# strawberrylady99/mythril

Measured on AMD Instinct MI355X. Metric: candidate assignments evaluated/sec (node) + time-to-first-model vs z3, higher is better.
Workload: dtype u32

## Files before the change

mythril_amd/csrc/jit_asm.cpp:

```cpp
#include <algorithm>
#include <array>
#include <cstdio>
#include <cstring>
#include <functional>
#include <map>
#include <set>
#include <sstream>
#include <string>
#include <vector>

#include "jit.hpp"

namespace mg {

namespace {

struct AsmFail {
  std::string why;
};
[[noreturn]] void fail(const std::string& w) { throw AsmFail{w}; }

inline uint32_t Lw(uint32_t w) { return (w + 31) / 32; }
inline uint32_t topmask(uint32_t w) { return (w & 31) ? ((1u << (w & 31)) - 1u) : 0xFFFFFFFFu; }
inline uint32_t gsalt(uint32_t c, uint32_t j) { return c * 0x9E3779B9u + j * 0x85EBCA6Bu + 0x27D4EB2Fu; }
// ... 134 lines not shown
  }
  std::function<bool()> on_pressure;
  std::function<bool()> on_hard;
  int vsoft = 256;
  int vhard = 256;
  uint32_t valloc() {
    for (;;) {
      int r = vfirst;
      while (r < vhard && vref[r]) r++;
      if ((r >= 256 || r >= vsoft) && on_pressure && on_pressure()) continue;
      if (r >= vhard && on_hard && on_hard()) continue;
      if (r >= vhard) fail("out of VGPRs");
      if (lds_pending.count(r)) lds_flush();
      vref[r] = 1;
      vgen[r] = ++gen_ctr;
      vhigh = std::max(vhigh, r + 1);
      return (uint32_t)r;
    }
  }
  uint32_t valloc2() {
    for (;;) {
      int r = (vfirst + 1) & ~1;
      while (r + 1 < vhard && (vref[r] || vref[r + 1])) r += 2;
      if ((r + 1 >= 256 || r + 1 >= vsoft) && on_pressure && on_pressure()) continue;
      if (r + 1 >= vhard && on_hard && on_hard()) continue;
      if (r + 1 >= vhard) fail("out of VGPRs");
      if (lds_pending.count(r) || lds_pending.count(r + 1)) lds_flush();
      for (int q = 0; q < 2; q++) {
        vref[r + q] = 1;
        vgen[r + q] = ++gen_ctr;
      }
      vhigh = std::max(vhigh, r + 2);
      return (uint32_t)r;
    }
  }
  void retain(const Limb& l) {
    check(l);
    if (l.reg() && (int)l.v >= vfirst) vref[l.v]++;
  }
  std::function<void(uint32_t)> on_free;
  void release(const Limb& l) {
    check(l);
    if (l.reg() && (int)l.v >= vfirst) {
      if (--vref[l.v] < 0) fail("internal: VGPR released twice");
      if (vref[l.v] == 0 && on_free) on_free(vgen[l.v]);
    }
  }
  int sfree() const {
    int n = 0;
    for (int r = kS0; r + 1 < kS1; r += 2) n += !sref[r];
    return n;
  }
  std::function<bool()> on_spressure;
  int salloc() {
    for (;;) {
      for (int r = kS0; r + 1 < kS1; r += 2)
        if (!sref[r]) {
          sref[r] = 1;
          shigh = std::max(shigh, r + 2);
          return r;
        }
      if (!on_spressure || !on_spressure()) break;
    }
    fail("out of SGPRs");
  }
  void sretain(const Mask& m) {
    if (m.k == 2) sref[m.s]++;
  }
  void srelease(const Mask& m) {
    if (m.k == 2 && --sref[m.s] < 0) fail("internal: SGPR pair released twice");
  }
};

struct Gen {
  const Lowered& P;
  const std::vector<GenSpec>& specs;
  const std::vector<uint32_t>& G;
  mutable Emitter E;
  std::vector<Val> val;
  std::vector<uint64_t> need;
  std::vector<int32_t> last;
  std::map<uint32_t, uint32_t> cval;
  std::vector<int32_t> def;
  std::vector<uint32_t> copysrc;
  bool gen_kernel = false;
  bool eval_kernel = false;
  std::map<uint32_t, uint32_t> lds_base;
  std::map<uint32_t, std::pair<uint32_t, uint32_t>> lds_shape;
  uint32_t lds_words = 0;
  static constexpr uint32_t kLdsWords = 8192;

  std::vector<Instr> code;
  Gen(const Lowered& p, const std::vector<GenSpec>& s, const std::vector<uint32_t>& g)
      : P(p), specs(s), G(g), val(p.vwidth.size()), need(p.vwidth.size(), 0), last(p.vwidth.size(), -1),
        def(p.vwidth.size(), -1), code(p.vcode) {}

  void reorder() {
    const std::vector<Instr>& v = P.vcode;
    std::vector<int32_t> dix(P.vwidth.size(), -1);
    for (size_t k = 0; k < v.size(); k++)
      if (v[k].dst != MG_NONE && v[k].dst < dix.size() && dix[v[k].dst] < 0) dix[v[k].dst] = (int32_t)k;
    std::map<uint32_t, int32_t> coord_at;
    for (size_t k = 0; k < v.size(); k++)
      if (v[k].op == K_COORD && !coord_at.count(v[k].p0)) coord_at[v[k].p0] = (int32_t)k;
    auto operands = [&](const Instr& in, std::vector<int32_t>& out) {
      out.clear();
      auto add = [&](uint32_t id) {
        if (id != MG_NONE && id < dix.size() && dix[id] >= 0) out.push_back(dix[id]);
      };
      switch (in.op) {
        case K_CONST: break;
// ... 508 lines not shown
      E.ctl("s_waitcnt vmcnt(0)");
      for (auto& pr : pend) {
        E.mem("ds_write_b32 " + VL(pr.second) + ", " + VL(pr.first));
        drop(pr.first);
        drop(pr.second);
      }
      pend.clear();
    };
    for (const auto& kv : lds_base) {
      const uint32_t off = kv.first, base = kv.second, n = lds_shape[off].first, Lc = lds_shape[off].second;
      const uint32_t nL = n * Lc, M = (65536u + Lc - 1) / Lc;
      for (uint32_t it = 0; it * 256 < nL; it++) {
        const Limb vi = fresh(), vt = fresh(), ve = fresh(), vj = fresh();
        E.valu("v_add_u32_e32 " + VL(vi) + ", " + imm(256 * it) + ", v0");
        E.valu("v_min_u32_e32 " + VL(vi) + ", " + imm(nL - 1) + ", " + VL(vi));
        E.valu("v_lshlrev_b32_e32 " + VL(vt) + ", 2, " + VL(vi));
        if (off * 4 < 4096) {
          E.mem("global_load_dword " + VL(vt) + ", " + VL(vt) + ", s[4:5] offset:" + std::to_string(off * 4));
        } else {
          E.valu("v_add_u32_e32 " + VL(vt) + ", " + hexs(off * 4) + ", " + VL(vt));
          E.mem("global_load_dword " + VL(vt) + ", " + VL(vt) + ", s[4:5]");
        }
        E.valu("v_mul_u32_u24_e32 " + VL(ve) + ", " + imm(M) + ", " + VL(vi));
        E.valu("v_lshrrev_b32_e32 " + VL(ve) + ", 16, " + VL(ve));
        E.valu("v_mul_u32_u24_e32 " + VL(vj) + ", " + imm(Lc) + ", " + VL(ve));
        E.valu("v_sub_u32_e32 " + VL(vj) + ", " + VL(vi) + ", " + VL(vj));
        if (lds_pairs()) {
          const Limb vo = fresh();
          E.valu("v_and_b32_e32 " + VL(vo) + ", 1, " + VL(vj));
          E.valu("v_and_b32_e32 " + VL(vj) + ", -2, " + VL(vj));
          E.valu("v_mul_u32_u24_e32 " + VL(vj) + ", " + imm(n) + ", " + VL(vj));
          E.valu("v_lshl_add_u32 " + VL(ve) + ", " + VL(ve) + ", 1, " + VL(vo));
          drop(vo);
        } else {
          E.valu("v_mul_u32_u24_e32 " + VL(vj) + ", " + imm(n) + ", " + VL(vj));
        }
        if (!inl(base)) E.salu("s_mov_b32 s41, " + hexs(base), {41});
        E.valu("v_add3_u32 " + VL(vj) + ", " + VL(vj) + ", " + VL(ve) + ", " + (inl(base) ? imm(base) : "s41"), {41});
        E.valu("v_lshlrev_b32_e32 " + VL(vj) + ", 2, " + VL(vj));
        drop(vi);
        drop(ve);
        pend.push_back({vt, vj});
        if (pend.size() >= stage_batch()) flush();
      }
    }
    flush();
    E.ctl("s_waitcnt lgkmcnt(0)");
    E.ctl("s_barrier");
  }

  Emitter& e() { return E; }

  int cond = 0;
  struct CondScope {
    Gen& g;
    explicit CondScope(Gen& g_) : g(g_) { g.cond++; }
    ~CondScope() { g.cond--; }
  };
  std::map<uint32_t, Limb> litcache;
  uint64_t tick = 0;
  std::map<uint32_t, uint64_t> lit_last;
  std::map<std::pair<uint64_t, uint64_t>, uint64_t> x_last;
  std::map<std::pair<uint32_t, uint32_t>, uint64_t> eq_last;
  void litcache_clear() {
    std::vector<Limb> held;
    for (auto& kv : litcache) held.push_back(kv.second);
    litcache.clear();
    lit_last.clear();
    for (auto& d : held) drop(d);
  }
  Limb vreg(const Limb& l) {
    if (l.reg()) {
      E.retain(l);
      return l;
    }
    const uint32_t x = l.lit() ? l.v : 0u;
    if (x == 0) return Reg(6);
    auto it = pool.find(x);
    if (it != pool.end()) return Reg((uint32_t)it->second);
    const bool cache = !cond && !no_lvn() && lvn_on && caches;
    if (cache) {
      auto c = litcache.find(x);
      if (c != litcache.end()) {
        lit_last[x] = ++tick;
        E.retain(c->second);
        return c->second;
      }
    }
    census[x]++;
    const Limb r = fresh();
    E.valu("v_mov_b32_e32 " + VL(r) + ", " + imm(x));
    if (cache) {
      E.retain(r);
      litcache[x] = r;
      lit_last[x] = ++tick;
    }
    return r;
  }
  bool lvn_on = false;
  bool caches = true;
  int vsoft = 256;
  std::map<uint32_t, int> pool;
  std::map<uint32_t, uint32_t> census;
  std::string src(const Limb& l) const {
    if (l.k == LU) fail("internal: a limb the demand analysis dropped was read");
    E.check(l);
    return l.lit() ? imm(l.v) : VL(l);
  }

// ... 279 lines not shown
    drop(c);
    return d;
  }

  static bool eq_bitop3() {
    static const bool on = [] {
      const char* g = getenv("MYTHGPU_JIT_ASM_EQ_BITOP3");
      return !(g && g[0] == '0');
    }();
    return on;
  }
  struct DLimb {
    uint32_t off = 0, n = 0, Lc = 0, j = 0;
    Limb idx;
  };
  std::map<uint32_t, DLimb> dlimb;
  static bool no_dict_eq() {
    static const bool on = [] {
      const char* g = getenv("MYTHGPU_JIT_ASM_NO_DICT_EQ");
      return g && g[0] == '1';
    }();
    return on;
  }
  void dlimb_free(uint32_t g) {
    auto it = dlimb.find(g);
    if (it == dlimb.end()) return;
    const Limb ix = it->second.idx;
    dlimb.erase(it);
    drop(ix);
  }
  bool dict_limb(const Limb& l, DLimb& out) const {
    if (!l.reg() || !l.g || (int)l.v < E.vfirst || E.vgen[l.v] != l.g) return false;
    auto it = dlimb.find(l.g);
    if (it == dlimb.end()) return false;
    out = it->second;
    return true;
  }
  bool idx_in_set(const Limb& idx, const std::vector<char>& S, uint32_t n, Mask& m) {
    uint32_t cnt = 0, first = 0, miss = 0;
    for (uint32_t e = 0; e < n; e++) {
      if (S[e]) {
        if (!cnt) first = e;
        cnt++;
      } else {
        miss = e;
      }
    }
    if (cnt == 0 || cnt == n) {
      m.k = 1;
      m.ones = cnt == n;
      return true;
    }
    if (cnt != 1 && cnt != n - 1 && n > 32) return false;
    m.k = 2;
    m.s = E.salloc();
    if (cnt == 1 || cnt == n - 1) {
      const uint32_t e = cnt == 1 ? first : miss;
      const std::string op = cnt == 1 ? "v_cmp_eq_u32" : "v_cmp_ne_u32";
      if (inl(e)) {
        E.valu(op + "_e64 " + SP(m.s) + ", " + imm(e) + ", " + VL(idx), {}, {m.s, m.s + 1});
      } else {
        E.valu(op + "_e32 vcc, " + hexs(e) + ", " + VL(idx), {}, {kVCC, kVCC + 1});
        E.salu("s_mov_b64 " + SP(m.s) + ", vcc", {m.s, m.s + 1});
      }
      return true;
    }
    uint32_t bits = 0;
    for (uint32_t e = 0; e < n; e++)
      if (S[e]) bits |= 1u << e;
    const Limb t = fresh();
    E.salu("s_mov_b32 s41, " + hexs(bits), {41});
    E.valu("v_bfe_u32 " + VL(t) + ", s41, " + VL(idx) + ", 1", {41});
    E.valu("v_cmp_ne_u32_e64 " + SP(m.s) + ", 0, " + VL(t), {}, {m.s, m.s + 1});
    drop(t);
    return true;
  }
  bool dict_eq(const std::vector<std::pair<Limb, Limb>>& prs, Mask& m) {
    if (no_dict_eq() || dlimb.empty()) return false;
    bool haveA = false, haveB = false;
    DLimb A, B;
    std::vector<std::pair<uint32_t, uint32_t>> lits;
    std::vector<std::pair<uint32_t, uint32_t>> regs;
    auto same_src = [](const DLimb& x, const DLimb& y) {
      return x.off == y.off && x.n == y.n && x.Lc == y.Lc && x.idx == y.idx && x.idx.g == y.idx.g;
    };
    for (const auto& pr : prs) {
      const Limb a = pr.first, b = pr.second;
      if (a.lit() && b.lit()) {
        if (a.v != b.v) {
          m.k = 1;
          m.ones = false;
          return true;
        }
        continue;
      }
      if (a == b) continue;
      DLimb da, db;
      const bool ia = dict_limb(a, da), ib = dict_limb(b, db);
      if ((ia && b.lit()) || (ib && a.lit())) {
        const DLimb& d = ia ? da : db;
        if (!haveA) {
          A = d;
          haveA = true;
        } else if (!same_src(A, d)) {
          return false;
        }
        lits.push_back({d.j, ia ? b.v : a.v});
      } else if (ia && ib) {
        if (!haveA) {
          A = da;
          haveA = true;
        }
        if (!haveB) {
          B = db;
          haveB = true;
        }
        const bool fwd = same_src(A, da) && same_src(B, db), rev = same_src(A, db) && same_src(B, da);
        if (!fwd && !rev) return false;
        const DLimb& x = fwd ? da : db;
        const DLimb& y = fwd ? db : da;
        regs.push_back({x.j, y.j});
      } else {
        return false;
      }
    }
    if (!haveA) return false;
    if (!lits.empty() && !regs.empty()) return false;
    if (!lits.empty()) {
      std::vector<char> S(A.n, 0);
      for (uint32_t e = 0; e < A.n; e++) {
        bool ok = true;
        for (const auto& lj : lits) ok = ok && G[A.off + e * A.Lc + lj.first] == lj.second;
        S[e] = ok;
      }
      return idx_in_set(A.idx, S, A.n, m);
    }
    if (!haveB || A.n != B.n || A.n > 256) return false;
    for (uint32_t e = 0; e < A.n; e++)
      for (uint32_t f = 0; f < B.n; f++) {
        bool eq = true;
        for (const auto& jj : regs) eq = eq && G[A.off + e * A.Lc + jj.first] == G[B.off + f * B.Lc + jj.second];
        if (eq != (e == f)) return false;
      }
    m.k = 2;
    m.s = E.salloc();
    E.valu("v_cmp_eq_u32_e64 " + SP(m.s) + ", " + VL(A.idx) + ", " + VL(B.idx), {}, {m.s, m.s + 1});
    return true;
  }
  Mask eq_mask(const std::vector<std::pair<Limb, Limb>>& prs, Limb* keep = nullptr) {
    {
      Mask dm;
      if (dict_eq(prs, dm)) return dm;
    }
    std::vector<Limb> diff;
    std::vector<std::pair<Limb, Limb>> raw;
    for (const auto& pr : prs) {
      const Limb a = pr.first, b = pr.second;
      if (a.lit() && b.lit()) {
        if (a.v != b.v) {
          for (auto& d : diff) drop(d);
          Mask m;
          m.k = 1;
          m.ones = false;
          return m;
        }
        continue;
      }
      if (a == b) continue;
      if (a.lit() && a.v == 0) {
        E.retain(b);
        diff.push_back(b);
        continue;
      }
      if (b.lit() && b.v == 0) {
        E.retain(a);
        diff.push_back(a);
        continue;
      }
      if (prs.size() == 1 || (diff.empty() && raw.empty() && &pr == &prs.back())) {
        const Limb s0 = b.reg() ? a : b, s1 = b.reg() ? b : a;
        Mask m;
        m.k = 2;
        m.s = E.salloc();
        if (s0.lit() && !inl(s0.v)) {
          E.valu("v_cmp_eq_u32_e32 vcc, " + src(s0) + ", " + VL(s1), {}, {kVCC, kVCC + 1});
          E.salu("s_mov_b64 " + SP(m.s) + ", vcc", {m.s, m.s + 1});
        } else {
          E.valu("v_cmp_eq_u32_e64 " + SP(m.s) + ", " + src(s0) + ", " + VL(s1), {}, {m.s, m.s + 1});
        }
        return m;
      }
      if (eq_bitop3()) {
        Limb hit;
        if (xcache_get(a, b, hit)) diff.push_back(hit);
        else raw.push_back({a, b});
      } else {
        diff.push_back(xor_limb(a, b));
      }
    }
// ... 94 lines not shown
  bool xcache_get(const Limb& a, const Limb& b, Limb& out) {
    if (!(lvn_on && caches && !cond && !no_lvn())) return false;
    const uint64_t k0 = lid(a), k1 = lid(b);
    auto it = xcache.find({std::min(k0, k1), std::max(k0, k1)});
    if (it == xcache.end()) return false;
    x_last[it->first] = ++tick;
    E.retain(it->second);
    out = it->second;
    return true;
  }
  void xcache_free(uint32_t g) {
    auto r = xby.equal_range(g);
    std::vector<std::pair<uint64_t, uint64_t>> keys;
    for (auto it = r.first; it != r.second; ++it) keys.push_back(it->second);
    xby.erase(r.first, r.second);
    for (const auto& k : keys) {
      auto it = xcache.find(k);
      if (it == xcache.end()) continue;
      const Limb d = it->second;
      xcache.erase(it);
      drop(d);
    }
  }
  void xcache_clear() {
    std::vector<Limb> held;
    for (auto& kv : xcache) held.push_back(kv.second);
    xcache.clear();
    xby.clear();
    for (auto& d : held) drop(d);
    for (auto& kv : hcache) drop(kv.second);
    hcache.clear();
    hby.clear();
    h_last.clear();
  }
  std::map<std::vector<uint64_t>, Limb> hcache;
  std::multimap<uint32_t, std::vector<uint64_t>> hby;
  std::map<std::vector<uint64_t>, uint64_t> h_last;
  void hcache_free(uint32_t g) {
    auto r = hby.equal_range(g);
    std::vector<std::vector<uint64_t>> keys;
    for (auto it = r.first; it != r.second; ++it) keys.push_back(it->second);
    hby.erase(r.first, r.second);
    for (const auto& k : keys) {
      auto it = hcache.find(k);
      if (it == hcache.end()) continue;
      const Limb d = it->second;
      hcache.erase(it);
      h_last.erase(k);
      drop(d);
    }
  }

  std::map<std::pair<uint32_t, uint32_t>, Limb> eqdiff;
  Mask eq_ids(uint32_t a, uint32_t b, uint32_t Lk) {
    PinScope pin_(*this, {a, b});
    const auto key = std::minmax(a, b);
    auto it = eqdiff.find(key);
    if (it != eqdiff.end()) {
      eq_last[key] = ++tick;
      Mask m;
      m.k = 2;
      m.s = E.salloc();
      E.valu("v_cmp_eq_u32_e64 " + SP(m.s) + ", 0, " + VL(it->second), {}, {m.s, m.s + 1});
      return m;
    }
    std::vector<std::pair<Limb, Limb>> prs;
    for (uint32_t j = 0; j < Lk; j++) prs.push_back({limb(a, j), limb(b, j)});
    Limb keep{};
    const Mask m = eq_mask(prs, &keep);
    if (keep.reg() && caches) {
      eqdiff[key] = keep;
      eq_last[key] = ++tick;
    }
    else if (keep.reg()) drop(keep);
    return m;
  }
  template <class M, class T>
  static typename M::iterator lru(M& m, T& last) {
    auto best = m.end();
    uint64_t bt = ~0ull;
    for (auto it = m.begin(); it != m.end(); ++it) {
      auto l = last.find(it->first);
      const uint64_t t = l == last.end() ? 0 : l->second;
      if (t < bt) {
        bt = t;
        best = it;
      }
    }
    return best;
  }
  bool evict_one() {
    if (!litcache.empty()) {
      auto it = lru(litcache, lit_last);
      const Limb d = it->second;
      lit_last.erase(it->first);
      litcache.erase(it);
      drop(d);
      return true;
    }
    if (!xcache.empty()) {
      auto it = lru(xcache, x_last);
      const Limb d = it->second;
      x_last.erase(it->first);
      xcache.erase(it);
      drop(d);
      return true;
    }
    if (!hcache.empty()) {
      auto it = lru(hcache, h_last);
      const Limb d = it->second;
      h_last.erase(it->first);
      hcache.erase(it);
      drop(d);
      return true;
    }
    if (!eqdiff.empty()) {
      auto it = lru(eqdiff, eq_last);
      const Limb d = it->second;
      eq_last.erase(it->first);
      eqdiff.erase(it);
      drop(d);
      return true;
    }
    return false;
  }
  size_t cur_k = 0;
  void note(const char* phase) {
    static const bool annotate = getenv("MYTHGPU_JIT_ASM_ANNOTATE") != nullptr;
    if (annotate) E.o << "  ; vcode " << cur_k << " " << phase << "\n";
  }
  bool spill_mask() {
    if (cur_k >= code.size()) return false;
    const Instr& in = code[cur_k];
    auto operand = [&](uint32_t id) {
      if (id == in.a || id == in.b || id == in.c) return true;
      if (in.op == K_LOOKUP) {
        if (id == in.p0) return true;
        for (uint32_t q = 0; q < 2 * in.c; q++)
          if (P.vaux[in.p1 + q] == id) return true;
      }
      return false;
    };
    int64_t best = -1;
    int32_t bl = -1;
    for (uint32_t id = 0; id < val.size(); id++) {
      const Val& x = val[id];
      if (!x.def || x.m.k != 2 || E.sref[x.m.s] != 1 || operand(id)) continue;
      const int32_t lu = id < last.size() ? last[id] : -1;
      if (lu > bl) {
        bl = lu;
        best = id;
      }
    }
    if (best < 0) return false;
    limb_of_bool((uint32_t)best);
    E.srelease(val[best].m);
    val[best].m = Mask{};
    return true;
  }
  void eq_forget(uint32_t id) {
    for (auto it = eqdiff.begin(); it != eqdiff.end();) {
      if (it->first.first == id || it->first.second == id) {
        drop(it->second);
        it = eqdiff.erase(it);
      } else {
        ++it;
      }
    }
  }

  static bool no_signed_lit() {
    static const bool on = [] {
      const char* g = getenv("MYTHGPU_JIT_ASM_NO_SIGNED_LIT");
      return g && g[0] == '1';
    }();
    return on;
  }
  static bool no_mulshare() {
    static const bool on = [] {
      const char* g = getenv("MYTHGPU_JIT_ASM_NO_MULSHARE");
      return g && g[0] == '1';
    }();
    return on;
  }
  static bool exit_skip() {
    static const bool on = [] {
      const char* g = getenv("MYTHGPU_JIT_ASM_EXIT_SKIP");
      return !(g && g[0] == '0');
    }();
    return on;
  }
  static bool no_slt_clamp() {
    static const bool on = [] {
      const char* g = getenv("MYTHGPU_JIT_ASM_NO_SLT_CLAMP");
      return g && g[0] == '1';
    }();
    return on;
  }
  Limb clamp32(const std::vector<Limb>& rv, uint32_t La, uint32_t tb) {
    if (!(lvn_on && caches && !cond && !no_lvn())) return Limb{};
    std::vector<uint64_t> key{0xC1A3Full, tb};
    for (uint32_t j = 0; j < La; j++) {
      if (rv[j].reg() && (int)rv[j].v >= E.vfirst && !rv[j].g) return Limb{};
      key.push_back(lid(rv[j]));
    }
    auto it = hcache.find(key);
    if (it != hcache.end()) {
// ... 2614 lines not shown
      case K_LOOKUP: {
        const uint32_t Lk = Lw(in.b), n = in.c;
        auto key_test = [&](uint32_t kv) -> Mask {
          if (!no_eq_cache()) return eq_ids(in.a, kv, Lk);
          std::vector<std::pair<Limb, Limb>> prs;
          for (uint32_t j = 0; j < Lk; j++) prs.push_back({limb(in.a, j), limb(kv, j)});
          return eq_mask(prs);
        };
        if (in.wd == 1 && !no_bool_lookup()) {
          Mask cur = mask_of(in.p0);
          E.sretain(cur);
          for (int32_t p = (int32_t)n - 1; p >= 0; p--) {
            const uint32_t kv = P.vaux[in.p1 + 2 * p], vv = P.vaux[in.p1 + 2 * p + 1];
            const Mask h = key_test(kv);
            if (h.k == 1) {
              if (h.ones) {
                E.srelease(cur);
                cur = mask_of(vv);
                E.sretain(cur);
              }
              continue;
            }
            const Mask vm = mask_of(vv);
            Mask nc;
            if (cur.k == 1 && !cur.ones) {
              nc = mop("and", h, vm);
            } else if (cur.k == 1 && vm.k == 2) {
              nc.k = 2;
              nc.s = E.salloc();
              E.salu("s_orn2_b64 " + SP(nc.s) + ", " + SP(vm.s) + ", " + SP(h.s), {nc.s, nc.s + 1});
            } else if (cur.k == 1) {
              if (vm.ones) {
                nc.k = 1;
                nc.ones = true;
              } else {
                nc = mnot(h);
              }
            } else if (vm.k == 1) {
              nc = vm.ones ? mop("or", h, cur) : mop_andn(cur, h);
            } else {
              const Mask t = mop("and", h, vm);
              const Mask f = mop_andn(cur, h);
              nc = mop("or", t, f);
              E.srelease(t);
              E.srelease(f);
            }
            E.srelease(cur);
            E.srelease(h);
            cur = nc;
          }
          set_mask(d, cur);
          break;
        }
        if (n >= 2 && n <= 5 && !no_lookup_runs() && E.sfree() >= (int)(n + n * (n - 1) / 2 + 4)) {
          std::vector<Mask> hs;
          std::vector<uint32_t> ps;
          int base = -1;
          for (int32_t p = (int32_t)n - 1; p >= 0; p--) {
            const Mask h = key_test(P.vaux[in.p1 + 2 * p]);
            if (h.k == 1) {
              if (h.ones) {
                for (auto& m : hs) E.srelease(m);
                hs.clear();
                ps.clear();
                base = p;
              }
              continue;
            }
            hs.push_back(h);
            ps.push_back((uint32_t)p);
          }
          const uint32_t dflt = base >= 0 ? P.vaux[in.p1 + 2 * base + 1] : in.p0;
          std::map<std::pair<size_t, size_t>, Mask> ors;
          auto run_mask = [&](size_t a, size_t b) -> Mask {
            if (a == b) return hs[a];
            auto it = ors.find({a, b});
            if (it != ors.end()) return it->second;
            const Mask prev = b - 1 == a ? hs[a] : ors.at({a, b - 1});
            const Mask m = mop("or", prev, hs[b]);
            ors[{a, b}] = m;
            return m;
          };
          std::vector<Limb> res(Ld);
          for (uint32_t j = 0; j < Ld; j++) {
            if (!(need[d] >> j & 1)) continue;
            Limb c = limb(dflt, j);
            E.retain(c);
            for (size_t a = 0; a < ps.size();) {
              const Limb v = limb(P.vaux[in.p1 + 2 * ps[a] + 1], j);
              size_t b = a;
              while (b + 1 < ps.size() && limb(P.vaux[in.p1 + 2 * ps[b + 1] + 1], j) == v) b++;
              if (!(v == c)) {
                for (size_t q = a + 1; q < b; q++) run_mask(a, q);
                const Mask m = run_mask(a, b);
                const Limb t = v3(v), f = v3(c);
                const Limb r = fresh();
                E.valu("v_cndmask_b32_e64 " + VL(r) + ", " + src(f) + ", " + src(t) + ", " + SP(m.s), {m.s, m.s + 1});
                drop(t);
                drop(f);
                drop(c);
                c = r;
              }
              a = b + 1;
            }
            res[j] = c;
          }
          for (auto& kv : ors) E.srelease(kv.second);
// ... 124 lines not shown
    static const bool on = [] {
      const char* g = getenv("MYTHGPU_JIT_ASM_NO_BOOL_LOOKUP");
      return g && g[0] == '1';
    }();
    return on;
  }
  static bool no_eq_cache() {
    static const bool on = [] {
      const char* g = getenv("MYTHGPU_JIT_ASM_NO_EQ_CACHE");
      return g && g[0] == '1';
    }();
    return on;
  }
  static bool gen_only() {
    static const bool on = [] {
      const char* g = getenv("MYTHGPU_JIT_ASM_GEN_ONLY");
      return g && g[0] == '1';
    }();
    return on;
  }
  static bool debug_live() {
    static const bool on = getenv("MYTHGPU_JIT_ASM_DEBUG") != nullptr;
    return on;
  }
  void operands_of(const Instr& in, size_t k, std::vector<uint32_t>& out) {
    std::function<void(uint32_t)> add = [&](uint32_t id) {
      if (id == MG_NONE || id >= val.size()) return;
      out.push_back(id);
      if (is_view(id)) {
        const Instr& vi = code[def[id]];
        add(vi.a);
        if (vi.op == K_CONCAT) add(vi.b);
      }
    };
    switch (in.op) {
      case K_CONST: break;
      case K_COORD: if (copysrc[k] != MG_NONE) add(copysrc[k]); break;
      case K_LOOKUP:
        add(in.a);
        add(in.p0);
        for (uint32_t q = 0; q < in.c; q++) add(P.vaux[in.p1 + 2 * q + 1]);
        break;
      default:
        add(in.a);
        if (in.op != K_NOT && in.op != K_NEG && in.op != K_EXTRACT && in.op != K_ZEXT && in.op != K_SEXT &&
            in.op != K_ASSERT && in.op != K_COPY && in.op != K_WATCH)
          add(in.b);
        if (in.op == K_ITE) add(in.c);
        break;
    }
  }
  void body(const std::string& next) {
    eqdiff.clear();
    mulshare.clear();
    xcache.clear();
    xby.clear();
    hcache.clear();
    hby.clear();
    h_last.clear();
    litcache.clear();
    lit_last.clear();
    x_last.clear();
    eq_last.clear();
    dlimb.clear();
    E.on_free = [this](uint32_t g) {
      xcache_free(g);
      hcache_free(g);
      dlimb_free(g);
    };
    E.on_pressure = [this]() { return evict_one(); };
    E.on_hard = [this]() { return spill_one(); };
    spill_at.assign(val.size(), {});
    slot_busy.clear();
    pinned.clear();
    E.on_spressure = [this]() { return spill_mask(); };
    lvn_on = true;
    static const bool annotate = getenv("MYTHGPU_JIT_ASM_ANNOTATE") != nullptr;
    for (size_t k = 0; k < code.size(); k++) {
      const Instr& in = code[k];
      cur_k = k;
      if (is_view(in.dst)) continue;
      if (annotate)
        E.o << "  ; vcode " << k << " op " << in.op << " w " << in.wd << " dst " << in.dst << " a " << in.a << " b " << in.b
            << "\n";
      if (spill_on) {
        pinned.clear();
        operands_of(in, k, pinned);
        for (size_t q = 0; q < pinned.size(); q++)
          if (is_spilled(pinned[q])) reload(pinned[q]);
      }
      emit(in, k, next);
      if (spill_on) pinned.clear();
      if (debug_live()) {
        int used = 0;
        for (int r = E.vfirst; r < 256; r++) used += E.vref[r] > 0;
        fprintf(stderr, "asm live %zu op %u w %u: %d VGPRs\n", k, in.op, in.wd, used);
        static const long at = getenv("MYTHGPU_JIT_ASM_DEBUG_AT") ? atol(getenv("MYTHGPU_JIT_ASM_DEBUG_AT")) : -1;
        if ((long)k == at) {
          std::map<uint32_t, int> byop;
          for (uint32_t id = 0; id < val.size(); id++) {
            if (!val[id].def) continue;
            int regs = 0;
            for (const auto& l : val[id].l) regs += l.reg();
            if (regs && def[id] >= 0) byop[code[def[id]].op] += regs;
          }
          for (const auto& kv : byop) fprintf(stderr, "  live from op %u: %d limbs\n", kv.first, kv.second);
        }
      }
      auto done = [&](uint32_t id) {
        if (id != MG_NONE && id < last.size() && last[id] <= (int32_t)k && val[id].def) {
          kill(id);
          val[id].def = false;
          if (!eqdiff.empty()) eq_forget(id);
        }
      };
      if (in.dst != MG_NONE && in.dst < last.size() && last[in.dst] < 0) done(in.dst);
      switch (in.op) {
        case K_CONST: break;
        case K_WATCH:
          if (eval_kernel) done(in.a);
          break;
        case K_COORD:
          if (copysrc[k] != MG_NONE) done(copysrc[k]);
          break;
        case K_LOOKUP:
          done(in.a);
          done(in.p0);
          for (uint32_t q = 0; q < 2 * in.c; q++) done(P.vaux[in.p1 + q]);
          break;
        default:
          done(in.a);
          if (in.b != MG_NONE) done(in.b);
          if (in.op == K_ITE) done(in.c);
          if (in.op == K_CONCAT || in.op == K_EXTRACT) {
            std::function<void(uint32_t)> through = [&](uint32_t id) {
              if (!is_view(id)) return;
              const Instr& vi = code[def[id]];
              done(vi.a);
              through(vi.a);
              if (vi.op == K_CONCAT) {
                done(vi.b);
                through(vi.b);
              }
            };
            through(in.a);
            if (in.op == K_CONCAT) through(in.b);
          }
          break;
      }
    }
    for (auto& kv : mulshare)
      for (auto& t : kv.second) drop(t);
    mulshare.clear();
    for (auto& kv : eqdiff) drop(kv.second);
    eqdiff.clear();
    xcache_clear();
    litcache_clear();
    lvn_on = false;
    E.on_free = nullptr;
    E.on_pressure = nullptr;
    E.on_hard = nullptr;
    E.on_spressure = nullptr;
  }

  bool sgkey = false;
  static int sgkey_env() {
    static const int v = [] {
      const char* g = getenv("MYTHGPU_JIT_ASM_SGKEY");
      return g ? (g[0] == '1' ? 1 : 0) : -1;
    }();
    return v;
  }
  bool salu_group_key() const { return sgkey; }
  void sfmix(int x) {
    auto xs = [&]() {
      E.salu("s_lshr_b32 s40, " + S(x + 1) + ", 1", {40});
      E.salu("s_xor_b32 " + S(x) + ", " + S(x) + ", s40", {x});
    };
    auto mul = [&](uint32_t clo, uint32_t chi) {
      E.salu("s_mul_hi_u32 s40, " + S(x) + ", " + hexs(clo), {40});
      E.salu("s_mul_i32 s41, " + S(x) + ", " + hexs(chi), {41});
      E.salu("s_add_u32 s40, s40, s41", {40});
      E.salu("s_mul_i32 s41, " + S(x + 1) + ", " + hexs(clo), {41});
      E.salu("s_add_u32 " + S(x + 1) + ", s40, s41", {x + 1});
      E.salu("s_mul_i32 " + S(x) + ", " + S(x) + ", " + hexs(clo), {x});
    };
    xs();
    mul(0xED558CCDu, 0xFF51AFD7u);
    xs();
    mul(0x1A85EC53u, 0xC4CEB9FEu);
    xs();
  }
  void vfmix(int lo, int hi) {
    const Limb t1 = fresh(), t2 = fresh();
    auto xs = [&]() {
      E.valu("v_lshrrev_b32_e32 " + VL(t1) + ", 1, " + V(hi));
      E.valu("v_xor_b32_e32 " + V(lo) + ", " + V(lo) + ", " + VL(t1));
    };
    auto mul = [&](uint32_t clo, uint32_t chi) {
      E.salu("s_mov_b32 s40, " + hexs(clo), {40});
      E.salu("s_mov_b32 s41, " + hexs(chi), {41});
      E.valu("v_mul_hi_u32 " + VL(t1) + ", " + V(lo) + ", s40", {40});
      E.valu("v_mul_lo_u32 " + VL(t2) + ", " + V(lo) + ", s41", {41});
      E.valu("v_add_u32_e32 " + VL(t1) + ", " + VL(t1) + ", " + VL(t2));
      E.valu("v_mul_lo_u32 " + VL(t2) + ", " + V(hi) + ", s40", {40});
      E.valu("v_add_u32_e32 " + V(hi) + ", " + VL(t1) + ", " + VL(t2));
      E.valu("v_mul_lo_u32 " + V(lo) + ", " + V(lo) + ", s40", {40});
    };
// ... 310 lines not shown
      E.salu("s_cmp_lt_u32 s16, s8");
      E.ctl("s_cbranch_scc0 " + exit_);
    }
    E.valu("v_add_u32_e32 v3, s16, v1", {16});
    if (tiled) {
      E.salu("s_lshr_b32 s30, s16, 6", {30});
      if (solo) E.salu("s_min_u32 s30, s30, s31", {30});
      block_base(26, 30);
      E.salu("s_add_u32 s33, s30, s32", {33});
      E.salu("s_min_u32 s33, s33, s31", {33});
      block_base(28, 33);
      page_at[0] = page_at[1] = -1;
    } else {
      E.valu("v_min_u32_e32 v2, s23, v3", {23});
      E.valu("v_lshlrev_b32_e32 v2, 2, v2");
      E.valu("v_add_u32_e32 " + VL(vnext) + ", s17, v3", {17});
      E.valu("v_min_u32_e32 " + VL(vnext) + ", s23, " + VL(vnext), {23});
      E.valu("v_lshlrev_b32_e32 " + VL(vnext) + ", 2, " + VL(vnext));
    }
    E.valu("v_cmp_gt_u32_e64 s[24:25], s8, v3", {8}, {24, 25});
    E.valu("v_lshlrev_b32_e32 v8, 2, v3");
    E.salu("s_mov_b64 s[38:39], -1", {38, 39});
    rows_issued = ring_reg.size();
    rows_used = 0;
    loads = 0;
    for (size_t q = 0; q < ring_reg.size(); q++) row_seq[q] = (long)q - (long)ring_reg.size();
    if (glds) {
      for (size_t q = 0; q < gdepth; q++) gseq[q] = (long)q - (long)gdepth;
      gl_issued = gdepth;
      staged = 0;
      lgkm_n = 0;
    }
    body("");
    if (rows_used != rows.size()) fail("internal: SoA rows left unread");
    if (glds && (gl_issued != rows.size() + gdepth || staged != rows.size())) fail("internal: LDS row queue");
    for (const Limb& l : ring_reg) drop(l);
    if (!tiled) drop(vnext);
    if (glds) drop(glds_v);
    if (spill_on) drop(spill_v);
    ring_reg.clear();
    for (int r = E.vfirst; r < 256; r++)
      if (E.vref[r]) fail("internal: VGPR v" + std::to_string(r) + " still held after the body");
    E.valu("v_cndmask_b32_e64 v7, 0, 1, s[38:39]", {38, 39});
    E.salu("s_mov_b64 exec, s[24:25]");
    E.mem("global_store_byte v3, v7, s[10:11]");
    E.salu("s_mov_b64 exec, -1");
    if (!solo) {
      E.salu("s_add_u32 s16, s16, s17", {16});
      E.ctl("s_branch " + loop);
    }
    E.label(exit_);
    E.ctl("s_waitcnt vmcnt(0)");
    E.ctl("s_endpgm");
    const int nv = std::max(E.vhigh, kV0), ns = std::max(E.shigh, rp_used ? 102 : 56);
    const int accum = (nv + 3) / 4 * 4;
    o << "  .section .rodata,\"a\",@progbits\n  .p2align 6, 0x0\n  .amdhsa_kernel " << name << "\n"
      << "    .amdhsa_group_segment_fixed_size " << eval_lds_bytes() << "\n    .amdhsa_private_segment_fixed_size 0\n"
      << "    .amdhsa_kernarg_size 36\n"
      << "    .amdhsa_user_sgpr_count 2\n    .amdhsa_user_sgpr_kernarg_segment_ptr 1\n"
      << "    .amdhsa_system_sgpr_workgroup_id_x 1\n    .amdhsa_system_vgpr_workitem_id 0\n"
      << "    .amdhsa_next_free_vgpr " << nv << "\n    .amdhsa_next_free_sgpr " << ns << "\n"
      << "    .amdhsa_accum_offset " << accum << "\n    .amdhsa_reserve_vcc 1\n"
      << "    .amdhsa_float_denorm_mode_32 3\n    .amdhsa_float_denorm_mode_16_64 3\n"
      << "  .end_amdhsa_kernel\n";
    if (solo)
      o << "  .globl mgj_meta_eval_cpb\n  .p2align 2\n  .type mgj_meta_eval_cpb,@object\nmgj_meta_eval_cpb:\n"
           "  .long 64\n  .size mgj_meta_eval_cpb, 4\n";
    o << "  .text\n";
    labels = E.nlab;
    meta_vgpr[name] = nv;
    meta_sgpr[name] = ns + 6;
    std::string res = o.str();
    if (spill_on) {
      const size_t at = res.find("__MG_SPILL_BYTES__");
      if (at != std::string::npos) res.replace(at, 18, hexs(spill_stride() * 256u));
      const size_t st = res.find("__MG_SPILL_STRIDE_");
      if (st != std::string::npos) res.replace(st, 18, hexs(spill_stride()));
    }
    return res;
  }

  uint32_t eval_lds_bytes() const {
    return (glds ? 4u * glds_slots() * 256u : 0u) + (spill_on ? (solo ? 1u : 4u) * spill_stride() * 256u : 0u);
  }

  int labels = 0;
  std::string kernel(const std::string& name) {
    E = Emitter();
    E.nlab = labels;
    E.vsoft = vsoft;
    census.clear();
    E.vfirst = kV0 + (int)pool.size();
    E.vhigh = E.vfirst;
    val.assign(P.vwidth.size(), Val{});
    cval.clear();
    auto& o = E.o;
    o << "  .text\n  .globl " << name << "\n  .p2align 8\n  .type " << name << ",@function\n" << name << ":\n";
    E.ctl("s_load_dwordx2 s[4:5], s[0:1], 0x0");
    E.ctl("s_load_dwordx8 s[8:15], s[0:1], 0x8");
    if (gen_kernel) {
      E.ctl("s_load_dwordx2 s[16:17], s[0:1], 0x28");
      E.ctl("s_load_dword s19, s[0:1], 0x30");
    } else {
      E.ctl("s_load_dwordx4 s[16:19], s[0:1], 0x28");
    }
    E.valu("v_and_b32_e32 v1, 63, v0");
// ... 184 lines not shown
        E.ctl("s_waitcnt vmcnt(0)");
        E.valu("v_readfirstlane_b32 s50, v8", {}, {50});
        E.valu("v_readfirstlane_b32 s51, v9", {}, {51});
        E.valu("v_mov_b32_e32 v8, s46", {46});
        E.valu("v_mov_b32_e32 v9, s47", {47});
        E.mem("global_atomic_umin_x2 v6, v[8:9], s[50:51] sc1", {50, 51});
        E.salu("s_add_u32 s49, s49, 1", {49});
        E.salu("s_cmp_lt_u32 s49, s48");
        E.ctl("s_cbranch_scc1 " + ploop);
        E.label(pdone);
      }
      E.salu("s_mov_b64 exec, -1");
    }
    E.label(cont);
    E.salu("s_add_u32 s26, s26, s28", {26});
    E.salu("s_addc_u32 s27, s27, 0", {27});
    E.ctl("s_branch " + loop);
    E.label(exit_);
    if (!gen_kernel) {
      const std::string nobest = E.newlab(), end = E.newlab();
      E.salu("s_cmp_eq_u64 s[30:31], -1");
      E.ctl("s_cbranch_scc1 " + nobest);
      if (exit_skip()) {
        E.salu("s_mov_b64 exec, 1");
        E.mem("global_load_dwordx2 v[8:9], v6, s[16:17]", {16, 17});
        E.ctl("s_waitcnt vmcnt(0)");
        E.valu("v_readfirstlane_b32 s46, v8", {}, {46});
        E.valu("v_readfirstlane_b32 s47, v9", {}, {47});
        E.salu("s_mov_b64 exec, -1");
        E.salu("s_sub_u32 s44, s30, s46", {44});
        E.salu("s_subb_u32 s44, s31, s47", {44});
        E.ctl("s_cbranch_scc0 " + nobest);
      }
      E.salu("s_mov_b64 exec, 1");
      E.valu("v_mov_b32_e32 v8, s30", {30});
      E.valu("v_mov_b32_e32 v9, s31", {31});
      E.mem("global_atomic_umin_x2 v6, v[8:9], s[16:17]", {16, 17});
      E.salu("s_mov_b64 exec, -1");
      E.label(nobest);
      E.salu("s_cmp_eq_u64 s[32:33], 0");
      E.ctl("s_cbranch_scc1 " + end);
      E.salu("s_and_b32 s40, s2, 15", {40});
      E.salu("s_add_u32 s40, s40, 1", {40});
      E.salu("s_lshl_b32 s40, s40, 7", {40});
      E.salu("s_add_u32 s44, s16, s40", {44});
      E.salu("s_addc_u32 s45, s17, 0", {45});
      E.salu("s_mov_b64 exec, 1");
      E.valu("v_mov_b32_e32 v8, s32", {32});
      E.valu("v_mov_b32_e32 v9, s33", {33});
      E.mem("global_atomic_add_x2 v6, v[8:9], s[44:45]", {44, 45});
      E.label(end);
    }
    E.ctl("s_endpgm");
    static const int diag_vgprs = [] {
      const char* g = getenv("MYTHGPU_JIT_ASM_DIAG_VGPRS");
      return g ? std::max(0, std::min(256, atoi(g))) : 0;
    }();
    const int nv = std::max({E.vhigh, kV0, diag_vgprs}), ns = std::max(E.shigh, 56);
    const int accum = (nv + 3) / 4 * 4;
    o << "  .section .rodata,\"a\",@progbits\n  .p2align 6, 0x0\n  .amdhsa_kernel " << name << "\n"
      << "    .amdhsa_group_segment_fixed_size " << lds_words * 4 << "\n    .amdhsa_private_segment_fixed_size 0\n"
      << "    .amdhsa_kernarg_size " << (gen_kernel ? 52 : 56) << "\n"
      << "    .amdhsa_user_sgpr_count 2\n    .amdhsa_user_sgpr_kernarg_segment_ptr 1\n"
      << "    .amdhsa_system_sgpr_workgroup_id_x 1\n    .amdhsa_system_vgpr_workitem_id 0\n"
      << "    .amdhsa_next_free_vgpr " << nv << "\n    .amdhsa_next_free_sgpr " << ns << "\n"
      << "    .amdhsa_accum_offset " << accum << "\n    .amdhsa_reserve_vcc 1\n"
      << "    .amdhsa_float_denorm_mode_32 3\n    .amdhsa_float_denorm_mode_16_64 3\n"
      << "  .end_amdhsa_kernel\n  .text\n";
    labels = E.nlab;
    meta_lds = lds_words * 4;
    meta_vgpr[name] = nv;
    meta_sgpr[name] = ns + 6;
    return o.str();
  }
  std::map<std::string, int> meta_vgpr, meta_sgpr;
  uint32_t meta_lds = 0;
};

std::string metadata(const std::map<std::string, int>& vg, const std::map<std::string, int>& sg, bool with_gen,
                     uint32_t lds_bytes) {
  std::ostringstream o;
  auto arg = [&](uint32_t off, uint32_t size, const char* kind, bool global) {
    o << "      - .offset: " << off << "\n        .size: " << size << "\n        .value_kind: " << kind << "\n";
    if (global) o << "        .address_space: global\n";
  };
  o << "  .amdgpu_metadata\n---\namdhsa.kernels:\n";
  for (const char* name : {"mgj_search", "mgj_gen"}) {
    const bool gen = std::strcmp(name, "mgj_gen") == 0;
    if (gen && !with_gen) continue;
    o << "  - .args:\n";
    arg(0, 8, "global_buffer", true);
    for (uint32_t k = 0; k < 4; k++) arg(8 + 8 * k, 8, "by_value", false);
    arg(40, 8, "global_buffer", true);
    if (gen) {
      arg(48, 4, "by_value", false);
    } else {
      arg(48, 4, "by_value", false);
      arg(52, 4, "by_value", false);
    }
    o << "    .group_segment_fixed_size: " << lds_bytes << "\n    .kernarg_segment_align: 8\n"
      << "    .kernarg_segment_size: " << (gen ? 52 : 56) << "\n    .max_flat_workgroup_size: 256\n"
      << "    .name: " << name << "\n    .private_segment_fixed_size: 0\n"
      << "    .sgpr_count: " << sg.at(name) << "\n    .sgpr_spill_count: 0\n"
      << "    .symbol: " << name << ".kd\n    .uniform_work_group_size: 1\n    .uses_dynamic_stack: false\n"
      << "    .vgpr_count: " << vg.at(name) << "\n    .vgpr_spill_count: 0\n    .wavefront_size: 64\n"
      << "    .agpr_count: 0\n";
// ... 224 lines not shown
```

mythril_amd/csrc/program.cpp:

```cpp
#include "program.hpp"

#include <algorithm>
#include <cstring>
#include <functional>
#include <map>
#include <set>
#include <tuple>
#include <cstdio>
#include <cstdlib>

namespace mg {

static inline uint32_t L_of(uint32_t w) { return (w + 31) / 32; }

uint64_t op_cost(uint32_t k, uint32_t w, uint32_t wa) {
  const uint64_t L = L_of(w), La = L_of(wa);
  switch (k) {
    case K_ADD: case K_SUB: case K_NEG: case K_AND: case K_OR: case K_XOR: case K_NOT:
    case K_ITE: case K_EXTRACT: case K_CONCAT: case K_ZEXT: case K_SEXT:
      return L;
    case K_EQ: case K_ULT: case K_ULE: case K_SLT: case K_SLE:
      return 2 * La;
    case K_SHL: case K_LSHR: case K_ASHR:
      return 4 * L;
// ... 302 lines not shown
      }
      nl.p0 = eq_id(dflt);
      rep.push_back(std::move(nl));
    }
    if (single) drop[(size_t)defk[lk]] = 1;
    drop[k] = 1;
    at[k] = std::move(rep);
    *changed = true;
  }
  if (!*changed) return code;
  std::vector<VInstr> out;
  out.reserve(code.size() + 8);
  for (size_t k = 0; k < code.size(); k++) {
    if (!drop[k]) out.push_back(code[k]);
    for (auto& r : at[k]) out.push_back(std::move(r));
  }
  return out;
}

std::vector<VInstr> fold_not_compares(const std::vector<VInstr>& code, size_t nv, bool* changed) {
  std::vector<uint32_t> uses(nv, 0);
  std::vector<int64_t> def(nv, -1);
  for (size_t k = 0; k < code.size(); k++) {
    for_each_use(code[k], [&](uint32_t v) {
      if (v < nv) uses[v]++;
    });
    if (code[k].dst != MG_NONE && code[k].dst < nv) def[code[k].dst] = (int64_t)k;
  }
  std::vector<VInstr> out = code;
  std::vector<char> drop(code.size(), 0);
  for (size_t k = 0; k < code.size(); k++) {
    const VInstr& n = code[k];
    if (n.op != K_NOT || n.wd != 1 || n.a >= nv || uses[n.a] != 1 || def[n.a] < 0) continue;
    VInstr& c = out[def[n.a]];
    uint32_t op;
    switch (c.op) {
      case K_ULT: op = K_ULE; break;
      case K_ULE: op = K_ULT; break;
      case K_SLT: op = K_SLE; break;
      case K_SLE: op = K_SLT; break;
      default: continue;
    }
    c.op = op;
    std::swap(c.a, c.b);
    c.dst = n.dst;
    drop[k] = 1;
    *changed = true;
  }
  std::vector<VInstr> r;
  r.reserve(out.size());
  for (size_t k = 0; k < out.size(); k++)
    if (!drop[k]) r.push_back(std::move(out[k]));
  return r;
}

std::vector<VInstr> sink_inputs(const std::vector<VInstr>& code, size_t nv) {
  std::vector<int64_t> first(nv, -1);
  for (size_t k = 0; k < code.size(); k++)
    for_each_use(code[k], [&](uint32_t v) {
      if (v < nv && first[v] < 0) first[v] = (int64_t)k;
    });
  std::vector<std::vector<size_t>> before(code.size());
  std::vector<char> moved(code.size(), 0);
  for (size_t k = 0; k < code.size(); k++) {
    const VInstr& c = code[k];
    if ((c.op == K_COORD || c.op == K_CONST) && c.dst < nv && first[c.dst] > (int64_t)k) {
      before[(size_t)first[c.dst]].push_back(k);
      moved[k] = 1;
    }
  }
  std::vector<VInstr> out;
  out.reserve(code.size());
  for (size_t k = 0; k < code.size(); k++) {
    for (size_t m : before[k]) out.push_back(code[m]);
    if (!moved[k]) out.push_back(code[k]);
  }
  return out;
}

std::vector<VInstr> fuse_asserts(const std::vector<VInstr>& code, size_t nv) {
  static const bool on = [] {
    const char* g = getenv("MYTHGPU_INTERP_FUSE");
    return !(g && g[0] == '0');
  }();
  if (!on) return code;
  const uint32_t NONE = MG_NONE;
  std::vector<uint32_t> uses(nv, 0);
  std::vector<int64_t> user(nv, -1);
  auto use = [&](uint32_t v, size_t k) {
    if (v != NONE && v < nv) {
      uses[v]++;
      user[v] = (int64_t)k;
    }
  };
  for (size_t k = 0; k < code.size(); k++) {
    const VInstr& c = code[k];
    if (c.op == K_LOOKUP) {
      use(c.a, k);
      use(c.p0, k);
      for (uint32_t v : c.prior) use(v, k);
    } else if (c.op == K_CONCAT || c.op == K_EXTRACT || c.op == K_ZEXT || c.op == K_SEXT || c.op == K_KECCAK ||
               c.op == K_ASSERT || c.op == K_WATCH || c.op == K_COPY) {
      use(c.a, k);
      use(c.b, k);
    } else if (c.op != K_CONST && c.op != K_COORD) {
      use(c.a, k);
// ... 2024 lines not shown
        const bool side = (c.op == K_ASSERT && keep_asserts) || (c.op == K_WATCH && keep_watch);
        if (!side && (c.dst == NONE || c.dst >= nw || !live[c.dst])) continue;
        keep[k] = 1;
        auto use = [&](uint32_t x) {
          if (x != NONE && x < nw) live[x] = 1;
        };
        if (c.op == K_LOOKUP) {
          use(c.a);
          use(c.p0);
          for (uint32_t x : c.prior) use(x);
        } else if (c.op == K_CONCAT || c.op == K_EXTRACT || c.op == K_ZEXT || c.op == K_SEXT || c.op == K_KECCAK ||
                   c.op == K_ASSERT || c.op == K_WATCH || c.op == K_COPY) {
          use(c.a);
          use(c.b);
        } else if (c.op != K_CONST && c.op != K_COORD) {
          use(c.a);
          use(c.b);
          use(c.c);
        }
      }
      std::vector<VInstr> kept;
      kept.reserve(list.size());
      for (size_t k = 0; k < list.size(); k++)
        if (keep[k] && (keep_watch || list[k].op != K_WATCH)) kept.push_back(std::move(list[k]));
      return kept;
    };
    std::vector<VInstr> kept = dce(code);
    const uint64_t ops = in.limb_ops;
    out.limb_ops = 0;
    bool pushed = false, pruned = false, folded = false;
    static const bool fold_on = [] {
      const char* g = getenv("MYTHGPU_FOLD_NOT");
      return !(g && g[0] == '0');
    }();
    auto fold_nots = [&] { return fold_on; };
    auto jit_rewrites = [&](const std::vector<VInstr>& list) {
      std::vector<VInstr> r = prune_guarded_lookups(list, vwidth.size(), &pruned);
      if (pruned) r = dce(r);
      for (int round = 0; round < 4; round++) {
        bool again = false;
        r = push_eq_into_lookup(r, vwidth, out.consts, &again);
        if (!again) break;
        pushed = true;
        r = dce(r);
      }
      if (fold_nots()) r = fold_not_compares(r, vwidth.size(), &folded);
      return r;
    };
    const bool order = specs != nullptr;
    if (order) heavy_last(kept);
    if (narrowed) {
      std::vector<VInstr> kept_wide = jit_rewrites(dce(wide));
      if (order) heavy_last(kept_wide);
      allocate(kept_wide, vwidth, out, &kept);
    } else {
      std::vector<VInstr> jit_list = jit_rewrites(kept);
      if (order) heavy_last(jit_list);
      if (pushed || pruned || folded)
        allocate(jit_list, vwidth, out, &kept);
      else
        allocate(kept, vwidth, out);
    }
    out.limb_ops = ops;
    return MG_OK;
  } catch (const Fail& f) {
    err = f.msg;
    return f.code;
  } catch (const std::exception& e) {
    err = e.what();
    return MG_E_INVALID;
  }
}

}
```

Baseline: 268.3 billion.

## Cache comparison masks in SGPRs and add global value numbering pass

Adds a mask cache in the assembly JIT so equality and set-membership masks (eq_ids, dict_eq, idx_in_set) already computed into SGPR pairs are reused instead of recomputed. Cached pairs are evicted LRU under SGPR pressure, and some SGPR pairs are reserved before conditional scopes. A generation check guards against stale use. Separately adds a value-numbering pass over the IR that deduplicates identical pure instructions and repeated asserts before allocation. This removes redundant VALU compares and duplicate arithmetic in generated kernels, at the cost of longer SGPR live ranges and possible extra mask spills.

Measured after the change: 280.2 billion (median of 6 runs). 1.04x the previous value.

```diff
diff --git a/mythril_amd/csrc/jit_asm.cpp b/mythril_amd/csrc/jit_asm.cpp
--- a/mythril_amd/csrc/jit_asm.cpp
+++ b/mythril_amd/csrc/jit_asm.cpp
@@ -210,11 +210,20 @@
     return n;
   }
   std::function<bool()> on_spressure;
+  std::vector<uint32_t> sgen = std::vector<uint32_t>(kS1, 0);
+  uint32_t sgen_ctr = 0;
+  void scheck(int s, uint32_t tag) const {
+    if (!check_on()) return;
+    if (s < kS0 || s + 1 >= kS1 || sref[s] <= 0 || sgen[s] != tag)
+      fail("internal: cached mask s[" + std::to_string(s) + ":" + std::to_string(s + 1) +
+           "] used after its pair was released or reallocated");
+  }
   int salloc() {
     for (;;) {
       for (int r = kS0; r + 1 < kS1; r += 2)
         if (!sref[r]) {
           sref[r] = 1;
+          sgen[r] = ++sgen_ctr;
           shigh = std::max(shigh, r + 2);
           return r;
         }
@@ -829,9 +838,17 @@
   Emitter& e() { return E; }
 
   int cond = 0;
+  static constexpr int kCondPairs = 8;
+  void sreserve() {
+    while (E.sfree() < kCondPairs && E.on_spressure && E.on_spressure()) {
+    }
+  }
   struct CondScope {
     Gen& g;
-    explicit CondScope(Gen& g_) : g(g_) { g.cond++; }
+    explicit CondScope(Gen& g_) : g(g_) {
+      if (!g.cond) g.sreserve();
+      g.cond++;
+    }
     ~CondScope() { g.cond--; }
   };
   std::map<uint32_t, Limb> litcache;
@@ -1217,6 +1234,16 @@
       return true;
     }
     if (cnt != 1 && cnt != n - 1 && n > 32) return false;
+    MKey ck = idx_key(1, idx);
+    if (!ck.empty()) {
+      ck.push_back(n);
+      for (uint32_t e = 0; e < n; e += 64) {
+        uint64_t w = 0;
+        for (uint32_t q = e; q < n && q < e + 64; q++) w |= (uint64_t)(S[q] != 0) << (q - e);
+        ck.push_back(w);
+      }
+      if (mcache_get(ck, m)) return true;
+    }
     m.k = 2;
     m.s = E.salloc();
     if (cnt == 1 || cnt == n - 1) {
@@ -1228,6 +1255,7 @@
         E.valu(op + "_e32 vcc, " + hexs(e) + ", " + VL(idx), {}, {kVCC, kVCC + 1});
         E.salu("s_mov_b64 " + SP(m.s) + ", vcc", {m.s, m.s + 1});
       }
+      mcache_put(ck, m);
       return true;
     }
     uint32_t bits = 0;
@@ -1238,6 +1266,7 @@
     E.valu("v_bfe_u32 " + VL(t) + ", s41, " + VL(idx) + ", 1", {41});
     E.valu("v_cmp_ne_u32_e64 " + SP(m.s) + ", 0, " + VL(t), {}, {m.s, m.s + 1});
     drop(t);
+    mcache_put(ck, m);
     return true;
   }
   bool dict_eq(const std::vector<std::pair<Limb, Limb>>& prs, Mask& m) {
@@ -1307,9 +1336,23 @@
         for (const auto& jj : regs) eq = eq && G[A.off + e * A.Lc + jj.first] == G[B.off + f * B.Lc + jj.second];
         if (eq != (e == f)) return false;
       }
+    MKey ck = idx_key(2, A.idx);
+    {
+      const MKey kb = idx_key(2, B.idx);
+      if (kb.empty()) ck.clear();
+      if (!ck.empty()) {
+        ck.insert(ck.end(), kb.begin() + 1, kb.end());
+        if (std::make_pair(ck[3], ck[4]) < std::make_pair(ck[1], ck[2])) {
+          std::swap(ck[1], ck[3]);
+          std::swap(ck[2], ck[4]);
+        }
+        if (mcache_get(ck, m)) return true;
+      }
+    }
     m.k = 2;
     m.s = E.salloc();
     E.valu("v_cmp_eq_u32_e64 " + SP(m.s) + ", " + VL(A.idx) + ", " + VL(B.idx), {}, {m.s, m.s + 1});
+    mcache_put(ck, m);
     return true;
   }
   Mask eq_mask(const std::vector<std::pair<Limb, Limb>>& prs, Limb* keep = nullptr) {
@@ -1510,9 +1553,96 @@
   }
 
   std::map<std::pair<uint32_t, uint32_t>, Limb> eqdiff;
+
+  struct MEnt {
+    Mask m;
+    uint32_t tag = 0;
+    uint64_t used = 0;
+  };
+  typedef std::vector<uint64_t> MKey;
+  std::map<MKey, MEnt> mcache;
+  uint32_t mc_hits = 0, mc_evictions = 0, mc_spills = 0;
+  static bool no_mask_cache() {
+    static const bool off = [] {
+      const char* g = getenv("MYTHGPU_JIT_ASM_NO_MASK_CACHE");
+      return g && g[0] == '1';
+    }();
+    return off;
+  }
+  bool mcache_on() const { return lvn_on && caches && !cond && !no_mask_cache(); }
+  bool mcache_get(const MKey& key, Mask& m) {
+    if (key.empty() || !mcache_on()) return false;
+    auto it = mcache.find(key);
+    if (it == mcache.end()) return false;
+    E.scheck(it->second.m.s, it->second.tag);
+    it->second.used = ++tick;
+    m = it->second.m;
+    E.sretain(m);
+    mc_hits++;
+    return true;
+  }
+  void mcache_put(const MKey& key, const Mask& m) {
+    if (key.empty() || m.k != 2 || !mcache_on() || mcache.count(key)) return;
+    MEnt e;
+    e.m = m;
+    e.tag = E.sgen[m.s];
+    e.used = ++tick;
+    E.sretain(m);
+    mcache[key] = e;
+  }
+  bool mcache_evict() {
+    auto best = mcache.end();
+    for (auto it = mcache.begin(); it != mcache.end(); ++it)
+      if (best == mcache.end() || it->second.used < best->second.used) best = it;
+    if (best == mcache.end()) return false;
+    E.srelease(best->second.m);
+    mcache.erase(best);
+    mc_evictions++;
+    return true;
+  }
+  template <class F>
+  void mcache_drop_if(F&& f) {
+    for (auto it = mcache.begin(); it != mcache.end();) {
+      if (f(it->first)) {
+        E.srelease(it->second.m);
+        it = mcache.erase(it);
+      } else {
+        ++it;
+      }
+    }
+  }
+  void mcache_forget(uint32_t id) {
+    if (mcache.empty()) return;
+    mcache_drop_if([&](const MKey& k) { return k[0] == 0 && (k[1] == id || k[2] == id); });
+  }
+  void mcache_free(uint32_t g) {
+    if (mcache.empty()) return;
+    mcache_drop_if([&](const MKey& k) { return (k[0] == 1 && k[1] == g) || (k[0] == 2 && (k[1] == g || k[3] == g)); });
+  }
+  void mcache_note() {
+    E.o << "  ; mask cache: " << mc_hits << " hits, " << mc_evictions << " evictions, " << mc_spills << " mask spills\n";
+  }
+  int mcache_spare() const {
+    int n = 0;
+    for (const auto& kv : mcache) n += E.sref[kv.second.m.s] == 1;
+    return n;
+  }
+  MKey idx_key(uint64_t kind, const Limb& idx) const {
+    if (!idx.reg() || !idx.g || (int)idx.v < E.vfirst || E.vgen[idx.v] != idx.g) return {};
+    return MKey{kind, idx.g, idx.v};
+  }
+
   Mask eq_ids(uint32_t a, uint32_t b, uint32_t Lk) {
     PinScope pin_(*this, {a, b});
     const auto key = std::minmax(a, b);
+    const MKey mkey{0, key.first, key.second};
+    {
+      Mask hit;
+      if (mcache_get(mkey, hit)) {
+        if (eqdiff.count(key)) eq_last[key] = ++tick;
+        return hit;
+      }
+    }
     auto it = eqdiff.find(key);
     if (it != eqdiff.end()) {
       eq_last[key] = ++tick;
@@ -1520,6 +1650,7 @@
       m.k = 2;
       m.s = E.salloc();
       E.valu("v_cmp_eq_u32_e64 " + SP(m.s) + ", 0, " + VL(it->second), {}, {m.s, m.s + 1});
+      mcache_put(mkey, m);
       return m;
     }
     std::vector<std::pair<Limb, Limb>> prs;
@@ -1531,6 +1662,7 @@
       eq_last[key] = ++tick;
     }
     else if (keep.reg()) drop(keep);
+    mcache_put(mkey, m);
     return m;
   }
   template <class M, class T>
@@ -1588,7 +1720,7 @@
     if (annotate) E.o << "  ; vcode " << cur_k << " " << phase << "\n";
   }
   bool spill_mask() {
-    if (cur_k >= code.size()) return false;
+    if (cond || cur_k >= code.size()) return false;
     const Instr& in = code[cur_k];
     auto operand = [&](uint32_t id) {
       if (id == in.a || id == in.b || id == in.c) return true;
@@ -1611,6 +1743,7 @@
       }
     }
     if (best < 0) return false;
+    mc_spills++;
     limb_of_bool((uint32_t)best);
     E.srelease(val[best].m);
     val[best].m = Mask{};
@@ -4331,7 +4464,7 @@
           set_mask(d, cur);
           break;
         }
-        if (n >= 2 && n <= 5 && !no_lookup_runs() && E.sfree() >= (int)(n + n * (n - 1) / 2 + 4)) {
+        if (n >= 2 && n <= 5 && !no_lookup_runs() && E.sfree() + mcache_spare() >= (int)(n + n * (n - 1) / 2 + 4)) {
           std::vector<Mask> hs;
           std::vector<uint32_t> ps;
           int base = -1;
@@ -4562,6 +4695,8 @@
   }
   void body(const std::string& next) {
     eqdiff.clear();
+    mcache.clear();
+    mc_hits = mc_evictions = mc_spills = 0;
     mulshare.clear();
     xcache.clear();
     xby.clear();
@@ -4577,13 +4712,14 @@
       xcache_free(g);
       hcache_free(g);
       dlimb_free(g);
+      mcache_free(g);
     };
     E.on_pressure = [this]() { return evict_one(); };
     E.on_hard = [this]() { return spill_one(); };
     spill_at.assign(val.size(), {});
     slot_busy.clear();
     pinned.clear();
-    E.on_spressure = [this]() { return spill_mask(); };
+    E.on_spressure = [this]() { return mcache_evict() || spill_mask(); };
     lvn_on = true;
     static const bool annotate = getenv("MYTHGPU_JIT_ASM_ANNOTATE") != nullptr;
     for (size_t k = 0; k < code.size(); k++) {
@@ -4622,6 +4758,7 @@
           kill(id);
           val[id].def = false;
           if (!eqdiff.empty()) eq_forget(id);
+          mcache_forget(id);
         }
       };
       if (in.dst != MG_NONE && in.dst < last.size() && last[in.dst] < 0) done(in.dst);
@@ -4664,6 +4801,7 @@
     mulshare.clear();
     for (auto& kv : eqdiff) drop(kv.second);
     eqdiff.clear();
+    mcache_drop_if([](const MKey&) { return true; });
     xcache_clear();
     litcache_clear();
     lvn_on = false;
@@ -5080,6 +5218,7 @@
     E.label(exit_);
     E.ctl("s_waitcnt vmcnt(0)");
     E.ctl("s_endpgm");
+    mcache_note();
     const int nv = std::max(E.vhigh, kV0), ns = std::max(E.shigh, rp_used ? 102 : 56);
     const int accum = (nv + 3) / 4 * 4;
     o << "  .section .rodata,\"a\",@progbits\n  .p2align 6, 0x0\n  .amdhsa_kernel " << name << "\n"
@@ -5370,6 +5509,7 @@
       E.label(end);
     }
     E.ctl("s_endpgm");
+    mcache_note();
     static const int diag_vgprs = [] {
       const char* g = getenv("MYTHGPU_JIT_ASM_DIAG_VGPRS");
       return g ? std::max(0, std::min(256, atoi(g))) : 0;
diff --git a/mythril_amd/csrc/program.cpp b/mythril_amd/csrc/program.cpp
--- a/mythril_amd/csrc/program.cpp
+++ b/mythril_amd/csrc/program.cpp
@@ -378,6 +378,60 @@
   for (size_t k = 0; k < out.size(); k++)
     if (!drop[k]) r.push_back(std::move(out[k]));
   return r;
+}
+
+std::vector<VInstr> value_number(const std::vector<VInstr>& code, size_t nv) {
+  static const bool on = [] {
+    const char* g = getenv("MYTHGPU_GVN");
+    return !(g && g[0] == '0');
+  }();
+  if (!on) return code;
+  const uint32_t NONE = MG_NONE;
+  std::vector<uint32_t> rep(nv);
+  for (size_t v = 0; v < nv; v++) rep[v] = (uint32_t)v;
+  auto R = [&](uint32_t v) { return v != NONE && v < nv ? rep[v] : v; };
+  std::map<std::vector<uint32_t>, uint32_t> seen;
+  std::set<uint32_t> asserted;
+  std::vector<VInstr> out;
+  out.reserve(code.size());
+  for (const VInstr& c0 : code) {
+    VInstr c = c0;
+    if (c.op == K_LOOKUP) {
+      c.a = R(c.a);
+      c.p0 = R(c.p0);
+      for (uint32_t& v : c.prior) v = R(v);
+    } else if (c.op == K_CONCAT || c.op == K_EXTRACT || c.op == K_ZEXT || c.op == K_SEXT || c.op == K_KECCAK ||
+               c.op == K_ASSERT || c.op == K_WATCH || c.op == K_COPY) {
+      c.a = R(c.a);
+      c.b = R(c.b);
+    } else if (c.op != K_CONST && c.op != K_COORD) {
+      c.a = R(c.a);
+      c.b = R(c.b);
+      c.c = R(c.c);
+    }
+    if (c.op == K_ASSERT) {
+      if (!asserted.insert(c.a).second) continue;
+      out.push_back(std::move(c));
+      continue;
+    }
+    const bool pure = c.op != K_CONST && c.op != K_COORD && c.op != K_WATCH && c.op != K_ASSERT_CMP && c.dst != NONE &&
+                      c.dst < nv;
+    if (!pure) {
+      out.push_back(std::move(c));
+      continue;
+    }
+    if ((c.op == K_EQ || c.op == K_AND || c.op == K_OR || c.op == K_XOR || c.op == K_ADD || c.op == K_MUL) && c.a > c.b)
+      std::swap(c.a, c.b);
+    std::vector<uint32_t> key{c.op, c.wd, c.a, c.b, c.c, c.p0, c.op == K_LOOKUP ? 0u : c.p1};
+    key.insert(key.end(), c.prior.begin(), c.prior.end());
+    auto ins = seen.emplace(std::move(key), c.dst);
+    if (!ins.second) {
+      rep[c.dst] = ins.first->second;
+      continue;
+    }
+    out.push_back(std::move(c));
+  }
+  return out;
 }
 
 std::vector<VInstr> sink_inputs(const std::vector<VInstr>& code, size_t nv) {
@@ -2508,10 +2562,14 @@
     if (narrowed) {
       std::vector<VInstr> kept_wide = jit_rewrites(dce(wide));
       if (order) heavy_last(kept_wide);
+      kept_wide = value_number(kept_wide, vwidth.size());
+      kept = value_number(kept, vwidth.size());
       allocate(kept_wide, vwidth, out, &kept);
     } else {
       std::vector<VInstr> jit_list = jit_rewrites(kept);
       if (order) heavy_last(jit_list);
+      jit_list = value_number(jit_list, vwidth.size());
+      kept = value_number(kept, vwidth.size());
       if (pushed || pruned || folded)
         allocate(jit_list, vwidth, out, &kept);
       else
```
